# B3zaleel/draco-sharp

Hardware: AMD Instinct MI355X
Metric: decoded_meshes_per_sec (higher is better)
Workload: dtype int32

## Files before the change

### draco-sharp_amd/csrc/dsa_api.hip

```cpp
#include <hip/hip_runtime.h>
#include <atomic>
#include <mutex>

#include <cstdarg>
#include <cstdio>
#include <cstring>
#include <memory>
#include <new>
#include <string>
#include <vector>

#include "../../include/draco_mi355x.h"
#include "dsa_kernels.h"
#include "dsa_seams.h"
#include "dsa_general.h"
#include "dsa_host_parse.h"
#include "dsa_host_util.h"

namespace {

enum { STG_LOCATE = 0, STG_CONNECTIVITY, STG_TRAVERSE, STG_OPERANDS, STG_SYMBOLS, STG_PREDICT, STG_FINALIZE, STG_TOTAL };
static const char *kStageNames[DSA_NUM_STAGES] = {"locate", "connectivity", "traverse", "para_operands",
                                                 "symbols", "predict", "finalize", "total"};
enum { KT_CHAIN = 0, KT_CONNECTIVITY, KT_TRAVERSE, KT_SYMBOLS_EARLY, KT_SYMBOLS_LATE, KT_OCT_STREAMS, KT_PREDICT_WRAP_EARLY, KT_PREDICT_WRAP_LATE, KT_FACES,
       KT_SEAM_TABLES, KT_TRAVERSE_ATT, KT_TEXCOORDS, KT_COUNT };
static const char *kKernelNames[KT_COUNT] = {"k_chain", "k_connectivity", "k_traverse", "k_symbols_reg[early]", "k_symbols_reg[late]", "k_predict_oct_streams",
                                             "k_predict_wrap[early]", "k_predict_wrap[late]", "k_faces", "k_seam_tables", "k_traverse_att", "k_texcoords"};


}

struct EncLane {
  int device = 0;
  hipStream_t st = nullptr;
  hostutil::Staging stage[2];
  int next = 0;
  hostutil::UploadTurns *upload_turn = nullptr;
  uint32_t upload_chunk = 0;
  hipStream_t walk_st = nullptr;
  hipEvent_t tables_done = nullptr, walk_done = nullptr;
  hipEvent_t seams_done = nullptr;
  struct Buf {
    void *p = nullptr; uint64_t cap = 0;
    hipError_t ensure(uint64_t bytes) {
      if (bytes <= cap) return hipSuccess;
      if (p) (void)hipFree(p);
      p = nullptr; cap = 0;
      const uint64_t want = bytes + bytes / 4;
      hipError_t e = hipMalloc(&p, want);
      if (e != hipSuccess) { (void)hipGetLastError(); p = nullptr; e = hipMalloc(&p, bytes); if (e == hipSuccess) cap = bytes; else p = nullptr; return e; }
      cap = want;
      return hipSuccess;
    }
    ~Buf() { if (p) (void)hipFree(p); }
  } arena, streams, conns, seams, packed, items;
  ~EncLane() {
    if (walk_st) { (void)hipStreamSynchronize(walk_st); (void)hipStreamDestroy(walk_st); }
    if (st) { (void)hipStreamSynchronize(st); (void)hipStreamDestroy(st); }
    if (tables_done) (void)hipEventDestroy(tables_done);
    if (walk_done) (void)hipEventDestroy(walk_done);
    if (seams_done) (void)hipEventDestroy(seams_done);
  }
};

struct StreamSet {
  hipStream_t stream = nullptr;
  hipStream_t stream2 = nullptr;
  hipStream_t stream3 = nullptr;
  hipStream_t stream4 = nullptr;
  hipStream_t stream5 = nullptr;
  hipEvent_t ev_join3 = nullptr, ev_trav = nullptr, ev_maps = nullptr, ev_early = nullptr, ev_flips = nullptr;
  hipEvent_t ev_fork = nullptr, ev_join = nullptr, ev_conn = nullptr;
  hipEvent_t ev_seambits = nullptr, ev_tables = nullptr, ev_att = nullptr;
  hipEvent_t ev_pred = nullptr;
  bool own_stream = false;
  hipError_t create(hipStream_t user, int least, int greatest) {
    hipError_t e = hipSuccess;
    if (user) { stream = user; own_stream = false; }
    else { e = hipStreamCreateWithPriority(&stream, hipStreamNonBlocking, greatest); own_stream = e == hipSuccess; }
    if (e == hipSuccess) e = hipStreamCreateWithPriority(&stream4, hipStreamNonBlocking, (least + greatest) / 2);
    if (e == hipSuccess) e = hipStreamCreateWithPriority(&stream2, hipStreamNonBlocking, least);
    if (e == hipSuccess) e = hipStreamCreateWithFlags(&stream3, hipStreamNonBlocking);
    if (e == hipSuccess) e = hipStreamCreateWithPriority(&stream5, hipStreamNonBlocking, least);
    for (hipEvent_t *ev : {&ev_join3, &ev_trav, &ev_maps, &ev_flips, &ev_early, &ev_fork, &ev_join, &ev_conn, &ev_seambits, &ev_tables, &ev_att, &ev_pred})
      if (e == hipSuccess) e = hipEventCreateWithFlags(ev, hipEventDisableTiming);
    return e;
  }
  void destroy() {
    for (hipEvent_t *ev : {&ev_join3, &ev_trav, &ev_maps, &ev_flips, &ev_early, &ev_fork, &ev_join, &ev_conn, &ev_seambits, &ev_tables, &ev_att, &ev_pred}) { if (*ev) (void)hipEventDestroy(*ev); *ev = nullptr; }
    for (hipStream_t *s : {&stream2, &stream3, &stream4, &stream5}) { if (*s) (void)hipStreamDestroy(*s); *s = nullptr; }
    if (own_stream && stream) (void)hipStreamDestroy(stream);
    stream = nullptr;
  }
};

struct dsa_context {
  int device = 0;
  StreamSet sets[2];
  int num_sets = 0;
  bool set1_made = false;
  int prio_least = 0, prio_greatest = 0;
  int last_set = 0;
  hipEvent_t last_done = nullptr;
  hipStream_t up = nullptr;
  hipStream_t down = nullptr;
  bool profiling = false;
  std::string err;
  hostutil::Staging stage[2];
  int stage_next = 0;
  struct Spare { uint8_t *p; uint64_t bytes; };
  std::vector<Spare> spare_arenas, spare_mirrors, spare_descs, spare_packed;
  static constexpr size_t kSpares = 3;
  std::atomic<int> live_batches{0};
  std::atomic<bool> doomed{false};
  std::mutex mu;
  std::vector<std::unique_ptr<EncLane>> enc_lanes;
  bool gate_ok = false;
  std::string gate_note;
};

struct dsa_batch {
  dsa_context *ctx = nullptr;
  uint32_t n = 0;
  std::vector<MeshLayout> layouts;
  std::vector<HostMesh> host;
  std::vector<MeshDesc> descs;
  uint8_t *arena = nullptr;
  uint64_t arena_bytes = 0, arena_cap = 0;
  MeshLayout *d_layouts = nullptr;
  MeshDesc *d_descs = nullptr;
  BatchGlobals *d_globals = nullptr;
  BatchGlobals globals = {};
  uint64_t out_base = 0, out_bytes = 0;
  uint64_t out_values = 0, out_values_bytes = 0;
  std::vector<CompactMesh> compact;
  CompactMesh *d_compact = nullptr;
  uint64_t packed_bytes = 0;
  uint8_t *d_packed = nullptr;
  uint64_t d_packed_cap = 0;
  bool mirror_compact = false;
  uint32_t max_faces = 0, max_vertices = 0, max_atts = 0, max_att_data = 0;
  uint64_t sum_vertices = 0;
  bool any_general = false, any_valence = false, any_seamed = false, any_multipara = false;
  bool decoded = false, collected = false;
  hipEvent_t ev[DSA_NUM_STAGES + 1] = {};
  hipEvent_t ev_sym[2] = {};
  hipEvent_t ev_k[KT_COUNT][2] = {};
  bool k_timed[KT_COUNT] = {};
  bool have_events = false;
  float stage_ms[DSA_NUM_STAGES] = {};
  float kernel_ms[KT_COUNT] = {};
  hipEvent_t ev_uploaded = nullptr, ev_done = nullptr, ev_descs = nullptr, ev_down = nullptr;
  MeshDesc *descs_pin = nullptr;
  uint64_t descs_pin_bytes = 0;
  uint8_t *mirror = nullptr;
  uint64_t mirror_bytes = 0;
  bool mirror_owned = false, download_queued = false, downloaded = false;
  bool all_general = false;
  dsa_batch *retry = nullptr;
  std::vector<int32_t> retry_index;
};

namespace {

dsa_status set_err(dsa_context *ctx, dsa_status st, const char *fmt, ...) {
  if (ctx) {
    char buf[512];
    va_list ap;
    va_start(ap, fmt);
    vsnprintf(buf, sizeof(buf), fmt, ap);
    va_end(ap);
// ... 176 lines not shown
  HIP_TRY(ctx, hipEventCreateWithFlags(&b->ev_done, hipEventDisableTiming));
  HIP_TRY(ctx, hipEventCreateWithFlags(&b->ev_descs, hipEventDisableTiming));
  HIP_TRY(ctx, hipEventCreateWithFlags(&b->ev_down, hipEventDisableTiming));
  {
    const uint64_t need = sizeof(MeshDesc) * (uint64_t)(n ? n : 1);
    uint8_t *p = take_spare(ctx, ctx->spare_descs, need, &b->descs_pin_bytes);
    if (!p) { HIP_TRY(ctx, hipHostMalloc((void **)&p, need + need / 2, hipHostMallocDefault)); b->descs_pin_bytes = need + need / 2; }
    b->descs_pin = (MeshDesc *)p;
  }
  {
    int turn;
    { std::lock_guard<std::mutex> g(ctx->mu); turn = ctx->stage_next; ctx->stage_next ^= 1; }
    hostutil::Staging &stg = ctx->stage[turn];
    HIP_TRY(ctx, stg.acquire(upload_bytes));
    uint8_t *h = stg.buf.p;
    if (n) memcpy(h + off_layouts, b->layouts.data(), sizeof(MeshLayout) * (size_t)n);
    memset(h + sizeof(MeshLayout) * (size_t)n, 0, (size_t)(off_globals - sizeof(MeshLayout) * (uint64_t)n));
    memcpy(h + off_globals, &b->globals, sizeof(BatchGlobals));
    const uint64_t first = n ? b->layouts[0].stream : upload_bytes;
    memset(h + off_globals + sizeof(BatchGlobals), 0, (size_t)(first - off_globals - sizeof(BatchGlobals)));
    if (n) memcpy(h + off_compact, b->compact.data(), sizeof(CompactMesh) * (size_t)n);
    hostutil::parallel_for(n, [&](uint32_t i) {
      const uint64_t at = b->layouts[i].stream, end = at + lengths[i], next = i + 1 < n ? b->layouts[i + 1].stream : upload_bytes;
      if (lengths[i]) memcpy(h + at, streams[i], lengths[i]);
      memset(h + end, 0, (size_t)(next - end));
    }, 8);
    HIP_TRY(ctx, hipMemcpyAsync(b->arena, h, upload_bytes, hipMemcpyHostToDevice, ctx->up));
    HIP_TRY(ctx, stg.submitted(ctx->up));
    HIP_TRY(ctx, hipEventRecord(b->ev_uploaded, ctx->up));
  }
  guard.b = nullptr;
  *out = b;
  return DSA_OK;
}

void gate_check(dsa_context *c) {
  hipFuncAttributes chain{}, reg{}, gate{};
  if (hipFuncGetAttributes(&chain, (const void *)dsa::k_chain) != hipSuccess || hipFuncGetAttributes(&reg, (const void *)dsa::k_symbols_reg) != hipSuccess ||
      hipFuncGetAttributes(&gate, (const void *)dsa::k_register_gate) != hipSuccess) {
    (void)hipGetLastError();
    c->gate_ok = false; c->gate_note = "k_register_gate left out: kernel attributes not available";
    return;
  }
  auto up8 = [](int r) { return (r + 7) / 8 * 8; };
  const int rc = up8(chain.numRegs), rr = up8(reg.numRegs), rg = up8(gate.numRegs), simd = 512;
  const int left = simd - 4 * rc - 3 * rr;
  c->gate_ok = left >= 0 && rg > left && rr > left && rg <= left + 3 * rr;
  char buf[256];
  snprintf(buf, sizeof(buf), "k_register_gate %s: registers k_chain %d, k_symbols_reg %d, k_register_gate %d; %d left beside 4 + 3 waves of a SIMD",
           c->gate_ok ? "in use" : "left out", chain.numRegs, reg.numRegs, gate.numRegs, left);
  c->gate_note = buf;
}

}

extern "C" {

int dsa_abi_version(void) { return DSA_ABI_VERSION; }

int dsa_device_count(void) {
  int n = 0;
  if (hipGetDeviceCount(&n) != hipSuccess) return 0;
  return n;
}

dsa_status dsa_context_create(int device, void *stream, dsa_context **out) {
  if (!out) return DSA_ERR_INVALID_ARGUMENT;
  *out = nullptr;
  int n = 0;
  if (hipGetDeviceCount(&n) != hipSuccess || device < 0 || device >= n) return DSA_ERR_DEVICE;
  dsa_context *c = new (std::nothrow) dsa_context();
  if (!c) return DSA_ERR_OUT_OF_MEMORY;
  c->device = device;
  if (hipSetDevice(device) != hipSuccess) { delete c; return DSA_ERR_DEVICE; }
  int least = 0, greatest = 0;
  (void)hipDeviceGetStreamPriorityRange(&least, &greatest);
  c->num_sets = stream ? 1 : 2;
  c->prio_least = least; c->prio_greatest = greatest;
  if (c->sets[0].create((hipStream_t)stream, least, greatest) != hipSuccess) { dsa_context_destroy(c); return DSA_ERR_DEVICE; }
  if (hipStreamCreateWithFlags(&c->up, hipStreamNonBlocking) != hipSuccess ||
      hipStreamCreateWithFlags(&c->down, hipStreamNonBlocking) != hipSuccess ||
      hipEventCreateWithFlags(&c->last_done, hipEventDisableTiming) != hipSuccess) { dsa_context_destroy(c); return DSA_ERR_DEVICE; }
  gate_check(c);
  *out = c;
  return DSA_OK;
}

void dsa_context_destroy(dsa_context *ctx) {
  if (!ctx) return;
  {
    std::lock_guard<std::mutex> g(ctx->mu);
    if (ctx->live_batches.load() > 0) { ctx->doomed = true; return; }
  }
  (void)hipSetDevice(ctx->device);
  if (ctx->up) { (void)hipStreamSynchronize(ctx->up); (void)hipStreamDestroy(ctx->up); }
  if (ctx->down) { (void)hipStreamSynchronize(ctx->down); (void)hipStreamDestroy(ctx->down); }
  drop_spares(ctx, ctx->spare_arenas, false);
  drop_spares(ctx, ctx->spare_packed, false);
  drop_spares(ctx, ctx->spare_mirrors, true);
  drop_spares(ctx, ctx->spare_descs, true);
  for (StreamSet &set : ctx->sets) set.destroy();
  if (ctx->last_done) (void)hipEventDestroy(ctx->last_done);
  delete ctx;
}

const char *dsa_last_error(const dsa_context *ctx) { return ctx ? ctx->err.c_str() : "null context"; }

dsa_status dsa_context_set_profiling(dsa_context *ctx, int enabled) {
  if (!ctx) return DSA_ERR_INVALID_ARGUMENT;
  ctx->profiling = enabled != 0;
  return DSA_OK;
}

#define DSA_GUARD(ctx, expr)                                                                              \
  try { return (expr); }                                                                                   \
  catch (const std::bad_alloc &) { return set_err((ctx), DSA_ERR_OUT_OF_MEMORY, "host allocation failed"); } \
  catch (...) { return set_err((ctx), DSA_ERR_DEVICE, "unexpected failure inside the library"); }

dsa_status dsa_batch_create(dsa_context *ctx, uint32_t n, const uint8_t *const *streams, const size_t *lengths, dsa_batch **out) {
  DSA_GUARD(ctx, build_batch(ctx, n, streams, lengths, out));
}

static dsa_status create_packed(dsa_context *ctx, uint32_t n, const uint8_t *blob, const uint64_t *offsets, dsa_batch **out) {
  std::vector<const uint8_t *> ptrs(n);
  std::vector<size_t> lens(n);
  for (uint32_t i = 0; i < n; ++i) {
    if (offsets[i + 1] < offsets[i]) return set_err(ctx, DSA_ERR_INVALID_ARGUMENT, "offsets must be non-decreasing");
    ptrs[i] = blob + offsets[i];
    lens[i] = (size_t)(offsets[i + 1] - offsets[i]);
  }
  return build_batch(ctx, n, ptrs.data(), lens.data(), out);
}
dsa_status dsa_batch_create_packed(dsa_context *ctx, uint32_t n, const uint8_t *blob, const uint64_t *offsets, dsa_batch **out) {
  if (!ctx || !out || (n && (!blob || !offsets))) return set_err(ctx, DSA_ERR_INVALID_ARGUMENT, "null argument");
  DSA_GUARD(ctx, create_packed(ctx, n, blob, offsets, out));
}

dsa_status dsa_batch_decode(dsa_batch *b) {
  if (!b) return DSA_ERR_INVALID_ARGUMENT;
  dsa_context *ctx = b->ctx;
  HIP_TRY(ctx, hipSetDevice(ctx->device));
  const uint32_t n = b->n;
  const bool was_decoded = b->decoded;
  b->decoded = true;
  b->collected = false;
  if (b->retry) { dsa_batch_free(b->retry); b->retry = nullptr; }
  b->retry_index.clear();
  int set_turn = 0;
  {
    std::lock_guard<std::mutex> g(ctx->mu);
    if (ctx->num_sets > 1 && ctx->last_done && hipEventQuery(ctx->last_done) == hipErrorNotReady) {
      set_turn = ctx->last_set ^ 1;
      if (set_turn == 1 && !ctx->set1_made) {
        if (ctx->sets[1].create(nullptr, ctx->prio_least, ctx->prio_greatest) == hipSuccess) ctx->set1_made = true;
        else { (void)hipGetLastError(); ctx->sets[1].destroy(); set_turn = 0; }
      }
    }
    (void)hipGetLastError();
    ctx->last_set = set_turn;
  }
  StreamSet &S = ctx->sets[set_turn];
  hipStream_t st = S.stream;
  if (n == 0) {
    HIP_TRY(ctx, hipEventRecord(b->ev_done, st));
    HIP_TRY(ctx, hipEventRecord(b->ev_descs, st));
    return DSA_OK;
  }
  const bool prof = ctx->profiling;
  if (prof && !b->have_events) {
    for (int i = 0; i <= DSA_NUM_STAGES; ++i) HIP_TRY(ctx, hipEventCreate(&b->ev[i]));
    for (int i = 0; i < 2; ++i) HIP_TRY(ctx, hipEventCreate(&b->ev_sym[i]));
    for (int k = 0; k < KT_COUNT; ++k) for (int i = 0; i < 2; ++i) HIP_TRY(ctx, hipEventCreate(&b->ev_k[k][i]));
    b->have_events = true;
  }
  for (int k = 0; k < KT_COUNT; ++k) b->k_timed[k] = false;
  auto k_begin = [&](int k, hipStream_t s) { if (prof && !b->k_timed[k]) (void)hipEventRecord(b->ev_k[k][0], s); };
  auto k_end = [&](int k, hipStream_t s) { if (prof && !b->k_timed[k]) { (void)hipEventRecord(b->ev_k[k][1], s); b->k_timed[k] = true; } };
  int evi = 0;
  auto mark = [&]() -> hipError_t { return prof ? hipEventRecord(b->ev[evi++], st) : hipSuccess; };
  if (b->download_queued && !b->downloaded) HIP_TRY(ctx, hipStreamWaitEvent(st, b->ev_down, 0));
  if (was_decoded) HIP_TRY(ctx, hipStreamWaitEvent(st, b->ev_done, 0));
  b->download_queued = false; b->downloaded = false;
  HIP_TRY(ctx, hipStreamWaitEvent(st, b->ev_uploaded, 0));
  HIP_TRY(ctx, hipMemsetAsync(b->d_descs, 0, sizeof(MeshDesc) * n, st));
  HIP_TRY(ctx, hipMemsetAsync(&b->d_globals->pool_cursor, 0, sizeof(unsigned long long) * 2, st));
  HIP_TRY(ctx, mark());
  {
    uint32_t gx = std::max<uint32_t>(1, std::min<uint32_t>((b->max_faces + 16383) / 16384, 4));
    hipLaunchKernelGGL(dsa::k_init, dim3(gx, n), dim3(256), 0, st, b->arena, b->d_layouts, n);
  }
  hipLaunchKernelGGL(dsa::k_locate, dim3(n), dim3(WAVE), 0, st, b->arena, b->d_layouts, b->d_descs, n, b->d_globals);
  for (uint32_t r = 0; r < std::max<uint32_t>(1, b->max_atts); ++r) {
    hipLaunchKernelGGL(dsa::k_tags, dim3(n), dim3(WAVE), 0, st, b->arena, b->d_layouts, b->d_descs, n);
    hipLaunchKernelGGL(dsa::k_locate_resume, dim3(n), dim3(WAVE), 0, st, b->arena, b->d_layouts, b->d_descs, n, b->d_globals);
  }
  if (b->any_valence) hipLaunchKernelGGL(dsa::k_valence_lists, dim3(n, 6), dim3(WAVE), 0, st, b->arena, b->d_layouts, b->d_descs, n);
  HIP_TRY(ctx, mark());
  const uint32_t na = std::max<uint32_t>(1, b->max_atts);
  static const bool serial = getenv("DSA_SERIAL") != nullptr;
#ifdef DSA_EXPERIMENTS
  auto env_int = [](const char *name, int dflt) { const char *e = getenv(name); return e ? atoi(e) : dflt; };
  static const int fuse_choice = env_int("DSA_FUSE_OPERANDS", -1), chain_choice = env_int("DSA_CHAIN", -1);
  static const uint32_t lane_flags = (uint32_t)env_int("DSA_LANES", (int)PW_FLAG);
  static const bool run_window = env_int("DSA_TRAV_NO_WINDOW", 0) == 0;
  static const int trav_split = env_int("DSA_TRAV_SPLIT", 1), split_mode = env_int("DSA_SYM_SPLIT", 1);
  static const uint32_t wide_flag = env_int("DSA_SYM_WIDE", 1) ? SYM_WIDE : 0u;
  static const bool early_fuse_on = env_int("DSA_EARLY_FUSE", 0) != 0;
  static const uint32_t oct_lpw = (uint32_t)env_int("DSA_OCT_LPW", 16);
  static const bool handoff_on = env_int("DSA_LATE_HANDOFF", 0) != 0;
#else
  const bool handoff_on = false;
  const int fuse_choice = -1, chain_choice = -1, trav_split = 1, split_mode = 1;
  const uint32_t lane_flags = PW_FLAG, wide_flag = SYM_WIDE;
  const bool run_window = true, early_fuse_on = false;
#endif
  const int oct_choice = []() { const char *e = getenv("DSA_OCT_STREAMS"); return e ? atoi(e) : -1; }();
  const bool oct_rule = n >= 3584 && (uint64_t)b->max_vertices * n <= 4 * b->sum_vertices;
  const uint32_t oct_flag = (oct_choice >= 0 ? oct_choice != 0 : oct_rule) && !(lane_flags & (LN_FLAG_OCT | LN_FLAG_PREDICT)) ? OS_FLAG : 0u;
  hipStream_t st2 = serial ? st : S.stream2, st3 = serial ? st : S.stream3;
  HIP_TRY(ctx, hipEventRecord(S.ev_fork, st));
  HIP_TRY(ctx, hipStreamWaitEvent(st2, S.ev_fork, 0));
  if (b->any_general) {
    HIP_TRY(ctx, hipStreamWaitEvent(st3, S.ev_fork, 0));
    hipLaunchKernelGGL(dsa::k_general, dim3(n), dim3(WAVE), 0, st3, b->arena, b->d_layouts, b->d_descs, n);
    hipLaunchKernelGGL(dsa::k_general_tables, dim3(n), dim3(WAVE), 0, st3, b->arena, b->d_layouts, b->d_descs, n);
    hipLaunchKernelGGL(dsa::k_general_attributes<0>, dim3(n), dim3(WAVE), 0, st3, b->arena, b->d_layouts, b->d_descs, n);
    hipLaunchKernelGGL(dsa::k_general_attributes<1>, dim3(n), dim3(WAVE), 0, st3, b->arena, b->d_layouts, b->d_descs, n);
    if (n > 2048) hipLaunchKernelGGL(dsa::k_general_values_crowded, dim3(n), dim3(WAVE), 0, st3, b->arena, b->d_layouts, b->d_descs, n);
    else hipLaunchKernelGGL(dsa::k_general_attributes<2>, dim3(n), dim3(WAVE), 0, st3, b->arena, b->d_layouts, b->d_descs, n);
    hipLaunchKernelGGL(dsa::k_general_attributes<3>, dim3(n), dim3(WAVE), 0, st3, b->arena, b->d_layouts, b->d_descs, n);
    HIP_TRY(ctx, hipEventRecord(S.ev_join3, st3));
  }
  if (!b->any_general) HIP_TRY(ctx, hipStreamWaitEvent(st3, S.ev_fork, 0));
  {
    uint32_t lpm = 1;
    while (lpm < b->max_att_data) lpm *= 2;
    const uint32_t per_wave = WAVE / lpm;
    hipLaunchKernelGGL(dsa::k_conn_checks, dim3((n + per_wave - 1) / per_wave), dim3(WAVE), 0, st3, b->arena, b->d_layouts, b->d_descs, n, lpm);
// ... 43 lines not shown
    k_end(KT_CONNECTIVITY, st);
    if (!b->any_seamed) HIP_TRY(ctx, launch_faces());
    if (b->any_seamed) {
      HIP_TRY(ctx, hipEventRecord(S.ev_trav, st));
      HIP_TRY(ctx, hipStreamWaitEvent(st3, S.ev_trav, 0));
      k_begin(KT_SEAM_TABLES, st3);
      hipLaunchKernelGGL(dsa::k_seam_tables, dim3(n), dim3(WAVE), 0, st3, b->arena, b->d_layouts, b->d_descs, n);
      k_end(KT_SEAM_TABLES, st3);
      for (uint32_t r = 0; r < std::max<uint32_t>(1, b->max_atts); ++r) {
        hipLaunchKernelGGL(dsa::k_tags, dim3(n), dim3(WAVE), 0, st3, b->arena, b->d_layouts, b->d_descs, n);
        hipLaunchKernelGGL(dsa::k_locate_resume, dim3(n), dim3(WAVE), 0, st3, b->arena, b->d_layouts, b->d_descs, n, b->d_globals);
      }
      HIP_TRY(ctx, hipEventRecord(S.ev_tables, st3));
      k_begin(KT_TRAVERSE_ATT, st3);
      hipLaunchKernelGGL(dsa::k_traverse_att, dim3(n, std::max<uint32_t>(1, b->max_att_data)), dim3(WAVE), 0, st3, b->arena, b->d_layouts, b->d_descs, n);
      k_end(KT_TRAVERSE_ATT, st3);
      HIP_TRY(ctx, hipEventRecord(S.ev_att, st3));
      HIP_TRY(ctx, launch_faces());
      {
        uint32_t lpm = 1;
        while (lpm < na) lpm *= 2;
        const uint32_t per_wave = WAVE / lpm;
        hipStream_t st5 = serial ? st : S.stream5;
        HIP_TRY(ctx, hipStreamWaitEvent(st5, S.ev_tables, 0));
        hipLaunchKernelGGL(dsa::k_flip_bits, dim3((n + per_wave - 1) / per_wave), dim3(WAVE), 0, st5, b->arena, b->d_layouts, b->d_descs, n, lpm, 1u);
        hipLaunchKernelGGL(dsa::k_orient_bits, dim3((n + per_wave - 1) / per_wave), dim3(WAVE), 0, st5, b->arena, b->d_layouts, b->d_descs, n, lpm, 1u);
        HIP_TRY(ctx, hipEventRecord(S.ev_flips, st5));
      }
    }
    HIP_TRY(ctx, mark());
    const uint32_t per = (n + (uint32_t)trav_split - 1) / (uint32_t)trav_split;
    k_begin(KT_TRAVERSE, st);
    for (uint32_t m0 = 0; m0 < n; m0 += per) {
      const uint32_t cnt = std::min(per, n - m0);
      hipLaunchKernelGGL(dsa::k_traverse, dim3(cnt), dim3(WAVE), 0, st, b->arena, b->d_layouts + m0, b->d_descs + m0, cnt, trav_flags);
    }
    k_end(KT_TRAVERSE, st);
    if (b->any_seamed) {
      HIP_TRY(ctx, launch_seam_maps());
    }
  }
  HIP_TRY(ctx, mark());
  if (prof) HIP_TRY(ctx, hipEventRecord(b->ev_sym[0], st2));
#ifdef DSA_EXPERIMENTS
  if (lane_flags & LN_FLAG_SYMBOLS) {
    const uint32_t groups = (n + WAVE - 1) / WAVE;
    hipLaunchKernelGGL(dsa::lanes::k_symbols_lanes<LN_T2_SYMS>, dim3(groups, na), dim3(WAVE), 0, st2, b->arena, b->d_layouts, b->d_descs, n, lane_flags);
    hipLaunchKernelGGL(dsa::lanes::k_symbols_lanes<LN_T1_SYMS>, dim3(groups, na), dim3(WAVE), 0, st2, b->arena, b->d_layouts, b->d_descs, n, lane_flags);
    hipLaunchKernelGGL(dsa::lanes::k_symbols_lanes<LN_T0_SYMS>, dim3(groups, na), dim3(WAVE), 0, st2, b->arena, b->d_layouts, b->d_descs, n, lane_flags);
  }
#endif
  const bool sym_split = !serial && !(lane_flags & (LN_FLAG_SYMBOLS | LN_FLAG_PREDICT)) && split_mode != 0;
  hipStream_t st4 = sym_split ? S.stream4 : st2;
  auto launch_symbols = [&](hipStream_t s, uint32_t fl, bool gate = false) {
    fl |= wide_flag;
    const uint32_t tier_blocks = (uint32_t)std::min<uint64_t>((uint64_t)n * na, SYM_TIER_BLOCKS);
    if (wide_flag) hipLaunchKernelGGL(dsa::k_symbols_wide, dim3(n, na), dim3(WAVE), 0, s, b->arena, b->d_layouts, b->d_descs, n, fl);
    hipLaunchKernelGGL(dsa::k_symbols<1>, dim3(tier_blocks), dim3(WAVE), dsa::sym_tier_lds_bytes(1), s, b->arena, b->d_layouts, b->d_descs, n, na, fl);
    hipLaunchKernelGGL(dsa::k_symbols<0>, dim3(tier_blocks), dim3(WAVE), dsa::sym_tier_lds_bytes(0), s, b->arena, b->d_layouts, b->d_descs, n, na, fl);
    hipLaunchKernelGGL(dsa::k_symbols<2>, dim3(tier_blocks), dim3(WAVE), dsa::sym_tier_lds_bytes(2), s, b->arena, b->d_layouts, b->d_descs, n, na, fl);
    if (gate) hipLaunchKernelGGL(dsa::k_register_gate, dim3(SYM_TIER_BLOCKS), dim3(WAVE), 0, s);
    const int kt = (fl & SYM_EARLY_ONLY) ? KT_SYMBOLS_EARLY : KT_SYMBOLS_LATE;
    k_begin(kt, s);
    hipLaunchKernelGGL(dsa::k_symbols_reg, dim3(n, na), dim3(WAVE), 0, s, b->arena, b->d_layouts, b->d_descs, n, fl);
    k_end(kt, s);
  };
  {
    const uint32_t gx = std::max<uint32_t>(1, std::min<uint32_t>((b->max_vertices + 16383) / 16384, 4));
    hipLaunchKernelGGL(dsa::k_point_maps, dim3(gx, n), dim3(256), 0, st2, b->arena, b->d_layouts, b->d_descs, n);
    HIP_TRY(ctx, hipEventRecord(S.ev_conn, st2));
  }
  const uint32_t early_fuse = early_fuse_on && !(lane_flags & (LN_FLAG_PREDICT | LN_FLAG_OCT)) ? SYM_EARLY_FUSE : 0u;
  const uint32_t hand = handoff ? LATE_HANDOFF : 0u;
  if (sym_split && split_mode == 2) {
    launch_symbols(st2, lane_flags | SYM_EARLY_ONLY | early_fuse);
    HIP_TRY(ctx, hipEventRecord(S.ev_conn, st2));
    HIP_TRY(ctx, hipStreamWaitEvent(st4, S.ev_conn, 0));
    launch_symbols(st2, lane_flags | SYM_LATE_ONLY | hand);
  } else if (sym_split && oct_flag) {
    HIP_TRY(ctx, hipStreamWaitEvent(st4, S.ev_conn, 0));
    launch_symbols(st4, lane_flags | SYM_EARLY_ONLY | early_fuse);
    launch_symbols(st2, lane_flags | SYM_LATE_ONLY | hand, ctx->gate_ok);
  } else if (sym_split) {
    HIP_TRY(ctx, hipStreamWaitEvent(st4, S.ev_conn, 0));
    launch_symbols(st4, lane_flags | SYM_EARLY_ONLY | early_fuse);
    launch_symbols(st2, lane_flags | SYM_LATE_ONLY | hand);
  } else launch_symbols(st2, lane_flags | early_fuse | hand);
  if (b->any_seamed) {
    HIP_TRY(ctx, hipEventRecord(S.ev_pred, st2));
    HIP_TRY(ctx, hipStreamWaitEvent(st2, S.ev_tables, 0));
    launch_symbols(st2, lane_flags | SYM_CORNER);
  }
  if (prof) HIP_TRY(ctx, hipEventRecord(b->ev_sym[1], st2));
  HIP_TRY(ctx, hipEventRecord(S.ev_join, st2));
#ifdef DSA_EXPERIMENTS
  if (lane_flags & LN_FLAG_PREDICT) hipLaunchKernelGGL(dsa::lanes::k_predict_lanes<16>, dim3((n + 15) / 16, na), dim3(WAVE), 0, st4, b->arena, b->d_layouts, b->d_descs, n, 0u);
  else
#endif
  {
    if (oct_flag) {
      k_begin(KT_OCT_STREAMS, st4);
      hipLaunchKernelGGL(dsa::k_predict_oct_streams, dim3((n + WAVE - 1) / WAVE, na), dim3(WAVE), OS_RING * 1024u, st4, b->arena, b->d_layouts, b->d_descs, n);
      k_end(KT_OCT_STREAMS, st4);
    }
    hipLaunchKernelGGL(dsa::k_predict, dim3(n, na), dim3(WAVE), 0, st4, b->arena, b->d_layouts, b->d_descs, n, 0u, lane_flags | oct_flag);
    if (lane_flags & PW_FLAG) {
      k_begin(KT_PREDICT_WRAP_EARLY, st4);
      hipLaunchKernelGGL(dsa::k_predict_wrap, dim3(n, na), dim3(WAVE), 0, st4, b->arena, b->d_layouts, b->d_descs, n, 0u, lane_flags);
      k_end(KT_PREDICT_WRAP_EARLY, st4);
    }
#ifdef DSA_EXPERIMENTS
    if (lane_flags & LN_FLAG_OCT) {
      if (oct_lpw == 8) hipLaunchKernelGGL(dsa::lanes::k_predict_oct_lanes<8>, dim3((n + 7) / 8, na), dim3(WAVE), 0, st4, b->arena, b->d_layouts, b->d_descs, n, lane_flags);
      else if (oct_lpw == 32) hipLaunchKernelGGL(dsa::lanes::k_predict_oct_lanes<32>, dim3((n + 31) / 32, na), dim3(WAVE), 0, st4, b->arena, b->d_layouts, b->d_descs, n, lane_flags);
      else if (oct_lpw == 64) hipLaunchKernelGGL(dsa::lanes::k_predict_oct_lanes<64>, dim3((n + 63) / 64, na), dim3(WAVE), 0, st4, b->arena, b->d_layouts, b->d_descs, n, lane_flags);
      else hipLaunchKernelGGL(dsa::lanes::k_predict_oct_lanes<16>, dim3((n + 15) / 16, na), dim3(WAVE), 0, st4, b->arena, b->d_layouts, b->d_descs, n, lane_flags);
    }
#endif
// ... 524 lines not shown
```

### draco-sharp_amd/csrc/dsa_kernels.h

```cpp
#pragma once
#include <hip/hip_runtime.h>
#include <stdint.h>

#include "dsa_common.h"
#include "dsa_locate.h"
#ifdef DSA_EXPERIMENTS
#include "dsa_lanes.h"
#else
#define LN_FLAG_SYMBOLS 1u
#define LN_FLAG_PREDICT 2u
#define LN_FLAG_OCT 8u
namespace dsa { namespace lanes {
__device__ __forceinline__ bool ln_sym_eligible(const AttrDesc &, const MeshLayout &, uint32_t, uint32_t) { return false; }
__device__ __forceinline__ bool ln_oct_eligible(const AttrDesc &, uint32_t) { return false; }
} }
#endif

#ifndef DSA_CHAIN_PRIO
#define DSA_CHAIN_PRIO 3
#endif

namespace dsa {

__device__ __forceinline__ uint32_t cnext(uint32_t c) { return (c % 3u == 2u) ? c - 2u : c + 1u; }
__device__ __forceinline__ uint32_t cprev(uint32_t c) { return (c % 3u == 0u) ? c + 2u : c - 1u; }
__device__ __forceinline__ uint32_t uni(uint32_t v) { return (uint32_t)__builtin_amdgcn_readfirstlane((int)v); }
__device__ __forceinline__ uint32_t lane_id() { return threadIdx.x & 63u; }
template <class T>
__device__ __forceinline__ T *uni_ptr(T *p) {
  const uint64_t v = (uint64_t)p;
  return (T *)(((uint64_t)(uint32_t)__builtin_amdgcn_readfirstlane((int)(uint32_t)(v >> 32)) << 32) | (uint32_t)__builtin_amdgcn_readfirstlane((int)(uint32_t)v));
}
__device__ __forceinline__ uint32_t rdlane(uint32_t v, uint32_t l) { return (uint32_t)__builtin_amdgcn_readlane((int)v, (int)l); }
#define SYM_WIDE 0x800u
#define SYM_EARLY_ONLY 0x100u
#define SYM_LATE_ONLY 0x200u
#define SYM_CORNER 0x1000u
#define PRED_FRONT 0x10000u
#define PRED_BEHIND 0x20000u
__device__ __forceinline__ bool att_behind_tables(const AttrDesc &a) { return a.corner_data != 0 || a.late_located != 0; }
__device__ __forceinline__ bool att_is_late(const AttrDesc &a) { return (a.have_scheme && a.pred_kind != 0) || att_behind_tables(a); }
#define PW_FLAG 4u
#define LATE_HANDOFF 0x40000u
__device__ __forceinline__ void late_handoff(uint8_t *arena, const MeshLayout &L, MeshDesc *D, uint32_t ai, uint32_t flags, uint32_t bit);
__device__ __forceinline__ bool pred_filtered(const AttrDesc &a, uint32_t flags) {
  return ((flags & PRED_FRONT) && att_behind_tables(a)) || ((flags & PRED_BEHIND) && !att_behind_tables(a));
}
__device__ __forceinline__ bool sym_filtered(const AttrDesc &a, uint32_t flags) {
  if (att_behind_tables(a)) return !(flags & SYM_CORNER);
  if (flags & SYM_CORNER) return true;
  const bool late = a.have_scheme && a.pred_kind != 0;
  return ((flags & SYM_EARLY_ONLY) && late) || ((flags & SYM_LATE_ONLY) && !late);
}
__device__ __forceinline__ uint64_t clk() { return __builtin_amdgcn_s_memtime(); }
__device__ __forceinline__ uint64_t realclk() { return __builtin_amdgcn_s_memrealtime(); }
__device__ __forceinline__ uint32_t leading_lanes(bool pred) { uint64_t m = ~__ballot(pred); return m ? (uint32_t)__builtin_ctzll(m) : 64u; }
#define WAIT_VM0() __builtin_amdgcn_s_waitcnt(0x0F70)

template <int CTRL>
__device__ __forceinline__ uint32_t dpp_mov(uint32_t x) { return (uint32_t)__builtin_amdgcn_update_dpp(0, (int)x, CTRL, 0xF, 0xF, false); }
__device__ __forceinline__ uint32_t lane_prev(uint32_t x) { return dpp_mov<0x138>(x); }
template <class Op>
__device__ __forceinline__ uint32_t wave_incl_scan(uint32_t x, Op op) {
  const uint32_t lane = lane_id(), rl = lane & 15u;
  uint32_t t;
  t = dpp_mov<0x111>(x); if (rl >= 1) x = op(t, x);
  t = dpp_mov<0x112>(x); if (rl >= 2) x = op(t, x);
  t = dpp_mov<0x114>(x); if (rl >= 4) x = op(t, x);
  t = dpp_mov<0x118>(x); if (rl >= 8) x = op(t, x);
  t = dpp_mov<0x142>(x); if ((lane & 31u) >= 16) x = op(t, x);
  t = dpp_mov<0x143>(x); if (lane >= 32) x = op(t, x);
  return x;
}
__device__ __forceinline__ uint32_t wave_excl_scan(uint32_t v, uint32_t *total) {
  const uint32_t x = wave_incl_scan(v, [](uint32_t a, uint32_t b) { return a + b; });
  *total = rdlane(x, 63);
  return x - v;
}

template <bool CP> struct Rec;
struct FaceIds { uint32_t v0, v1, v2, o0, o1, o2; };
template <> struct Rec<false> {
  static constexpr uint32_t WORDS = 8;
  struct Raw { uint4 v, o; };
  static __device__ __forceinline__ Raw load(const uint32_t *frec, uint32_t f) { Raw r; r.v = ((const uint4 *)frec)[(size_t)f * 2]; r.o = ((const uint4 *)frec)[(size_t)f * 2 + 1]; return r; }
// ... 1811 lines not shown
          }
        }
      } else {
        const uint32_t xs = uni((uint32_t)(P >> 32));
        mine = (lane == j) ? xs : mine;
        const uint32_t k5 = (xs >> 6) & 31u, l6 = xs & 63u;
        const uint32_t e0 = rdlane(tab_lo[k5], l6), e1 = rdlane(tab_hi[k5], l6);
        const uint32_t e = (xs & 2048u) ? e1 : e0;
        P = (uint64_t)((e & 0xFFFFu) * (xs >> 12) + (e >> 16)) << 32;
        ++j;
      }
    }
    if (lane < cnt) out[i0 + lane] = mine;
  }
  WAIT_VM0();
  __syncthreads();
  if (VLIST) {
    for (uint32_t i = lane; i < num_values; i += WAVE) out[i] = slot_sym[out[i] & 4095u];
    WAIT_VM0();
    __syncthreads();
    if (lane == 0) atomicOr(&D->val_lists_done, 1u << ai);
    return;
  }
  if (TAGS) {
    uint8_t *tags = arena + L.out[ai];
    uint64_t bits = 0;
    uint32_t worst = 0;
    const uint32_t nc = a.nc_portable;
    for (uint32_t i = lane; i < num_values; i += WAVE) {
      const uint32_t v = slot_sym[out[i] & 4095u];
      tags[i] = (uint8_t)v;
      bits += (uint64_t)v * nc;
      worst = v > worst ? v : worst;
    }
    for (int d = 32; d >= 1; d >>= 1) {
      bits += ((uint64_t)(uint32_t)__shfl_xor((int)(uint32_t)(bits >> 32), d, WAVE) << 32) | (uint32_t)__shfl_xor((int)(uint32_t)bits, d, WAVE);
      const uint32_t w2 = (uint32_t)__shfl_xor((int)worst, d, WAVE);
      worst = w2 > worst ? w2 : worst;
    }
    WAIT_VM0();
    __syncthreads();
    if (lane == 0) { a.table = (bits & 0x00FFFFFFFFFFFFFFull) | ((uint64_t)(worst > 255u ? 255u : worst) << 56); a.tags_done = 1; }
    return;
  }
  const bool positive = a.have_scheme && (a.pred_transform == 2 || a.pred_transform == 3);
  for (uint32_t i = lane; i < num_values; i += WAVE) {
    uint32_t v = slot_sym[out[i] & 4095u];
    out[i] = positive ? v : ((v & 1u) ? (uint32_t)(-(int32_t)(v >> 1) - 1) : (v >> 1));
  }
  early_tail(arena, L, D, ai, flags);
  late_handoff(arena, L, D, ai, flags, 1u);
}

__global__ __launch_bounds__(WAVE, 6) void k_symbols_reg(uint8_t *arena, const MeshLayout *layouts, MeshDesc *descs, uint32_t n, uint32_t flags) {
  uint32_t mesh = blockIdx.x, ai = blockIdx.y;
  if (mesh >= n) return;
  MeshDesc *D = &descs[mesh];
  if (D->status != ST_OK || D->general || ai >= D->num_attributes) return;
  reg_decode_stream<REG_ATTR>(arena, layouts[mesh], D, ai, flags);
}
__global__ __launch_bounds__(WAVE, 6) void k_tags(uint8_t *arena, const MeshLayout *layouts, MeshDesc *descs, uint32_t n) {
  uint32_t mesh = blockIdx.x;
  if (mesh >= n) return;
  MeshDesc *D = &descs[mesh];
  if (D->status != ST_OK || D->general || !D->values_pending || D->resume_att >= D->num_attributes) return;
  if (D->values_pending == 2) return;
  reg_decode_stream<REG_TAGS>(arena, layouts[mesh], D, D->resume_att, 0u);
}
__global__ __launch_bounds__(WAVE, 6) void k_valence_lists(uint8_t *arena, const MeshLayout *layouts, MeshDesc *descs, uint32_t n) {
  uint32_t mesh = blockIdx.x, c = blockIdx.y;
  if (mesh >= n) return;
  MeshDesc *D = &descs[mesh];
  if (D->status != ST_OK || D->general || D->encoder_type == 0 || D->traversal_type != 2) return;
  reg_decode_stream<REG_VLIST>(arena, layouts[mesh], D, c, 0u);
}

__device__ __forceinline__ bool sym_reg_eligible(const AttrDesc &a, const MeshLayout &L, uint32_t ai) {
  return a.source == SRC_RAW && a.precision_bits == 12 && a.num_symbols <= REG_MAX_SYMS && a.num_distinct > 1 &&
         L.out_cap[ai] >= 4096 * 6 + REG_MAX_SYMS * 4;
}
__device__ __forceinline__ bool sym_wide_eligible(const AttrDesc &a, const MeshLayout &L, uint32_t ai) {
  if (a.source != SRC_RAW || a.num_distinct <= 1 || sym_reg_eligible(a, L, ai)) return false;
  const bool compact = a.num_symbols > SYM_MAX_LDS;
  const uint32_t nse = compact ? a.num_distinct : a.num_symbols;
  if (nse <= 64 || nse > WIDE_MAX_SYMS || a.precision_bits > 16) return false;
  return compact ? (a.table != 0 && 2ull * nse + 1 <= (unsigned long long)a.num_symbols + 2) : (L.out_cap[ai] >= 4ull * (nse + 1));
}

__global__ __launch_bounds__(WAVE) void k_symbols_wide(uint8_t *arena, const MeshLayout *layouts, MeshDesc *descs, uint32_t n, uint32_t flags) {
  const uint32_t mesh = blockIdx.x, ai = blockIdx.y;
  if (mesh >= n) return;
  MeshDesc *D = &descs[mesh];
  if (D->status != ST_OK || D->general || ai >= D->num_attributes) return;
  const MeshLayout &L = layouts[mesh];
  const AttrDesc &a = D->att[ai];
  if (a.source == SRC_BYTES) return;
  if (lanes::ln_sym_eligible(a, L, ai, flags)) return;
  if (sym_filtered(a, flags)) return;
  if (!sym_wide_eligible(a, L, ai)) return;
  const uint32_t lane = lane_id();
  const uint32_t num_values = a.num_entries * a.nc_portable;
  if (num_values == 0) return;
  const uint8_t *stream = arena + L.stream;
  const uint32_t stream_len = L.stream_len;
  uint32_t *out = (uint32_t *)(arena + L.work[ai]);
  const bool compact = a.num_symbols > SYM_MAX_LDS;
  const uint32_t nsym = compact ? a.num_distinct : a.num_symbols;
  uint32_t *symtab = compact ? (uint32_t *)(arena + a.table) : nullptr;
  uint32_t *gtab = compact ? symtab + nsym : (uint32_t *)(arena + L.out[ai]);
  const uint32_t P = a.precision_bits, precision = 1u << P, l_base = precision * 4;
  if (lane == 0) {
    Rd r(stream, stream_len, a.off_table);
    uint32_t k = 0;
    bool ok = true;
    for (uint32_t i = 0; i < a.num_symbols && ok; ++i) {
      const uint32_t pd = r.u8(), token = pd & 3u;
      if (token == 3u) {
        const uint32_t offset = pd >> 2;
        if (i + offset >= a.num_symbols) ok = false;
        if (!compact) for (uint32_t j = 0; j <= offset && i + j < a.num_symbols; ++j) gtab[i + j] = 0;
        i += offset;
      } else {
        uint32_t pr = pd >> 2;
        for (uint32_t j = 0; j < token; ++j) pr |= r.u8() << (8 * (j + 1) - 2);
        if (compact) { if (pr) { if (k >= nsym) ok = false; else { gtab[k] = pr; symtab[k] = i; ++k; } } }
        else gtab[i] = pr;
      }
    }
    if (!ok || !r.ok || (compact && k != nsym)) fail(D, ST_INVALID, 400);
    WAIT_VM0();
    __threadfence_block();
  }
  __syncthreads();
// ... 1016 lines not shown
```

### draco-sharp_amd/csrc/dsa_types.h

```cpp
#pragma once
#include <stdint.h>

#define DSA_MAX_ATT 16
#define DSA_MAX_ATT_DATA 15
#define DSA_INVALID 0xFFFFFFFFu

#define ST_OK 0
#define ST_INVALID 1
#define ST_NOTIMPL 2
#define DSA_SITE_RETRY_GENERAL 170

#define SRC_TAGGED 0
#define SRC_RAW 1
#define SRC_FIXED 2
#define SRC_BYTES 3

struct AttrDesc {
  uint8_t att_type, data_type, nc, normalized;
  uint8_t seq_type;
  int8_t decoder_id;
  int8_t pred_method;
  int8_t pred_kind;
  int8_t pred_transform;
  uint8_t nc_portable;
// ... 147 lines not shown
  uint64_t total;
};
#if defined(__HIPCC__)
__host__ __device__
#endif
inline SeamLayout seam_layout(uint64_t F, uint64_t V, uint64_t A, bool compact) {
  SeamLayout g;
  const uint64_t NVA = 3 * F;
  uint64_t cur = 0;
  auto take = [&](uint64_t bytes) { uint64_t at = cur; cur = (cur + bytes + 16 + 255) & ~255ull; return at; };
  g.eseam = take(4 * F);
  g.vseam = take(V);
  g.pbase = take(4 * V);
  g.data = cur;
  cur = 0;
  g.bits = take(4 * ((3 * F / 2 + 31) / 32 + 4));
  g.rec = take((compact ? 16 : 32) * F);
  g.vbase = take(4 * V);
  g.vflag = take(NVA);
  g.d2c = take(4 * NVA);
  g.v2d = take(4 * NVA);
  g.fvis = take(F);
  g.stack = take(4 * F);
  g.para = take(12 * NVA);
  g.orient = take(4 * (NVA / 32 + 1));
  g.data_stride = cur;
  g.total = g.data + A * g.data_stride;
  return g;
}

struct MpPrep { uint32_t id[4][3]; };
#define MP_FOUND_SHIFT 29u
#define MP_ID_MASK 0x1FFFFFFFu

struct TcPrep {
  uint32_t next_id, prev_id;
  int64_t pn_norm2;
  int64_t cn_dot_pn;
  int64_t norm;
  double inv;
};

struct CompactMesh {
  uint64_t faces;
  uint32_t u16, pad;
  uint64_t map[DSA_MAX_ATT];
};

struct BatchGlobals {
  uint64_t pool;
  uint64_t pool_bytes;
  unsigned long long pool_cursor;
  unsigned long long pad;
};

struct MeshLayout {
  uint64_t stream;
  uint32_t stream_len;
  uint32_t cap_faces;
  uint32_t cap_vertices;
  uint32_t cap_attributes;
  uint64_t frec;
  uint64_t vrec;
  uint64_t d2c;
  uint64_t v2d;
  uint64_t fvis, vvis;
  uint64_t fstamp, vstamp;
  uint64_t splits;
  uint32_t cap_splits;
  uint32_t rec_compact;
  uint64_t vrank;
  uint64_t para;
  uint64_t faces;
  uint64_t work[DSA_MAX_ATT];
  uint64_t out[DSA_MAX_ATT];
  uint64_t map[DSA_MAX_ATT];
  uint32_t work_cap[DSA_MAX_ATT];
  uint32_t out_cap[DSA_MAX_ATT];
  uint64_t gen;
  uint64_t gen_bytes;
  uint32_t cap_points;
  uint32_t pad2;
  uint64_t seam;
  uint64_t seam_bytes;
  uint64_t tc[DSA_MAX_ATT];
  uint32_t mp_att;
  uint32_t pad_mp;
};
```

Before: 105,700.

## Add opt-in LDS-table rANS symbol decoder sharing work via atomic cursor

Adds a k_symbols_lds kernel that builds the rANS slot table in LDS and decodes streams one wave at a time. It runs on a new low-priority stream alongside k_symbols_reg, and both claim (mesh, attribute) items from a shared per-leg atomic cursor in BatchGlobals. The LDS path is gated by an environment variable plus register and LDS budget checks. The register decoder now always claims its work through the atomic cursor rather than using block indices, which adds one atomic per block and extra event waits.

```diff
diff --git a/draco-sharp_amd/csrc/dsa_api.hip b/draco-sharp_amd/csrc/dsa_api.hip
--- a/draco-sharp_amd/csrc/dsa_api.hip
+++ b/draco-sharp_amd/csrc/dsa_api.hip
@@ -69,10 +69,12 @@
   hipStream_t stream3 = nullptr;
   hipStream_t stream4 = nullptr;
   hipStream_t stream5 = nullptr;
+  hipStream_t stream6 = nullptr;
   hipEvent_t ev_join3 = nullptr, ev_trav = nullptr, ev_maps = nullptr, ev_early = nullptr, ev_flips = nullptr;
   hipEvent_t ev_fork = nullptr, ev_join = nullptr, ev_conn = nullptr;
   hipEvent_t ev_seambits = nullptr, ev_tables = nullptr, ev_att = nullptr;
   hipEvent_t ev_pred = nullptr;
+  hipEvent_t ev_lds[3] = {};
   bool own_stream = false;
   hipError_t create(hipStream_t user, int least, int greatest) {
     hipError_t e = hipSuccess;
@@ -82,13 +84,14 @@
     if (e == hipSuccess) e = hipStreamCreateWithPriority(&stream2, hipStreamNonBlocking, least);
     if (e == hipSuccess) e = hipStreamCreateWithFlags(&stream3, hipStreamNonBlocking);
     if (e == hipSuccess) e = hipStreamCreateWithPriority(&stream5, hipStreamNonBlocking, least);
-    for (hipEvent_t *ev : {&ev_join3, &ev_trav, &ev_maps, &ev_flips, &ev_early, &ev_fork, &ev_join, &ev_conn, &ev_seambits, &ev_tables, &ev_att, &ev_pred})
+    if (e == hipSuccess) e = hipStreamCreateWithPriority(&stream6, hipStreamNonBlocking, least);
+    for (hipEvent_t *ev : {&ev_join3, &ev_trav, &ev_maps, &ev_flips, &ev_early, &ev_fork, &ev_join, &ev_conn, &ev_seambits, &ev_tables, &ev_att, &ev_pred, &ev_lds[0], &ev_lds[1], &ev_lds[2]})
       if (e == hipSuccess) e = hipEventCreateWithFlags(ev, hipEventDisableTiming);
     return e;
   }
   void destroy() {
-    for (hipEvent_t *ev : {&ev_join3, &ev_trav, &ev_maps, &ev_flips, &ev_early, &ev_fork, &ev_join, &ev_conn, &ev_seambits, &ev_tables, &ev_att, &ev_pred}) { if (*ev) (void)hipEventDestroy(*ev); *ev = nullptr; }
-    for (hipStream_t *s : {&stream2, &stream3, &stream4, &stream5}) { if (*s) (void)hipStreamDestroy(*s); *s = nullptr; }
+    for (hipEvent_t *ev : {&ev_join3, &ev_trav, &ev_maps, &ev_flips, &ev_early, &ev_fork, &ev_join, &ev_conn, &ev_seambits, &ev_tables, &ev_att, &ev_pred, &ev_lds[0], &ev_lds[1], &ev_lds[2]}) { if (*ev) (void)hipEventDestroy(*ev); *ev = nullptr; }
+    for (hipStream_t *s : {&stream2, &stream3, &stream4, &stream5, &stream6}) { if (*s) (void)hipStreamDestroy(*s); *s = nullptr; }
     if (own_stream && stream) (void)hipStreamDestroy(stream);
     stream = nullptr;
   }
@@ -117,6 +120,8 @@
   std::vector<std::unique_ptr<EncLane>> enc_lanes;
   bool gate_ok = false;
   std::string gate_note;
+  bool lds_ok = false;
+  uint32_t lds_blocks = 0;
 };
 
 struct dsa_batch {
@@ -399,6 +404,27 @@
   c->gate_note = buf;
 }
 
+void lds_check(dsa_context *c) {
+  hipFuncAttributes chain{}, reg{}, lds{};
+  hipDeviceProp_t prop{};
+  c->lds_ok = false;
+  if (hipFuncGetAttributes(&chain, (const void *)dsa::k_chain) != hipSuccess || hipFuncGetAttributes(&reg, (const void *)dsa::k_symbols_reg) != hipSuccess ||
+      hipFuncGetAttributes(&lds, (const void *)dsa::k_symbols_lds) != hipSuccess || hipGetDeviceProperties(&prop, c->device) != hipSuccess) {
+    (void)hipGetLastError();
+    c->gate_note += "; k_symbols_lds left out: kernel attributes not available";
+    return;
+  }
+  auto up8 = [](int r) { return (r + 7) / 8 * 8; };
+  const int left = 512 - 4 * up8(chain.numRegs) - 3 * up8(reg.numRegs);
+  const long cu_lds = 160 * 1024, chain_lds = 16 * ((long)chain.sharedSizeBytes + CN_LDS_WORDS * 4), own_lds = 4 * ((long)lds.sharedSizeBytes + SL_LDS_BYTES);
+  c->lds_ok = up8(lds.numRegs) <= left && chain_lds + own_lds <= cu_lds && prop.multiProcessorCount > 0;
+  c->lds_blocks = 4u * (uint32_t)std::max(prop.multiProcessorCount, 1);
+  char buf[256];
+  snprintf(buf, sizeof(buf), "; k_symbols_lds %s: %d registers for %d left beside 4 + 3 waves of a SIMD, %ld + %ld bytes of LDS per CU", c->lds_ok ? "in use" : "left out",
+           lds.numRegs, left, chain_lds, own_lds);
+  c->gate_note += buf;
+}
+
 }
 
 extern "C" {
@@ -429,6 +455,7 @@
       hipStreamCreateWithFlags(&c->down, hipStreamNonBlocking) != hipSuccess ||
       hipEventCreateWithFlags(&c->last_done, hipEventDisableTiming) != hipSuccess) { dsa_context_destroy(c); return DSA_ERR_DEVICE; }
   gate_check(c);
+  lds_check(c);
   *out = c;
   return DSA_OK;
 }
@@ -530,7 +557,7 @@
   b->download_queued = false; b->downloaded = false;
   HIP_TRY(ctx, hipStreamWaitEvent(st, b->ev_uploaded, 0));
   HIP_TRY(ctx, hipMemsetAsync(b->d_descs, 0, sizeof(MeshDesc) * n, st));
-  HIP_TRY(ctx, hipMemsetAsync(&b->d_globals->pool_cursor, 0, sizeof(unsigned long long) * 2, st));
+  HIP_TRY(ctx, hipMemsetAsync(&b->d_globals->pool_cursor, 0, sizeof(BatchGlobals) - offsetof(BatchGlobals, pool_cursor), st));
   HIP_TRY(ctx, mark());
   {
     uint32_t gx = std::max<uint32_t>(1, std::min<uint32_t>((b->max_faces + 16383) / 16384, 4));
@@ -680,6 +707,12 @@
 #endif
   const bool sym_split = !serial && !(lane_flags & (LN_FLAG_SYMBOLS | LN_FLAG_PREDICT)) && split_mode != 0;
   hipStream_t st4 = sym_split ? S.stream4 : st2;
+  const int lds_choice = []() { const char *e = getenv("DSA_SYM_LDS"); return e ? atoi(e) : 0; }();
+  const bool lds_able = ctx->lds_ok && !early_fuse_on && !handoff_on && !(lane_flags & (LN_FLAG_SYMBOLS | LN_FLAG_PREDICT));
+  const bool lds_rule = n >= 3584 && chain && !serial && split_mode == 1;
+  const int sym_lds = !lds_able || lds_choice <= 0 ? 0 : lds_choice == 2 ? 2 : !lds_rule ? 0 : lds_choice == 3 ? 3 : 1;
+  hipStream_t st6 = serial ? st : S.stream6;
+  bool lds_forked = false;
   auto launch_symbols = [&](hipStream_t s, uint32_t fl, bool gate = false) {
     fl |= wide_flag;
     const uint32_t tier_blocks = (uint32_t)std::min<uint64_t>((uint64_t)n * na, SYM_TIER_BLOCKS);
@@ -688,10 +721,20 @@
     hipLaunchKernelGGL(dsa::k_symbols<0>, dim3(tier_blocks), dim3(WAVE), dsa::sym_tier_lds_bytes(0), s, b->arena, b->d_layouts, b->d_descs, n, na, fl);
     hipLaunchKernelGGL(dsa::k_symbols<2>, dim3(tier_blocks), dim3(WAVE), dsa::sym_tier_lds_bytes(2), s, b->arena, b->d_layouts, b->d_descs, n, na, fl);
     if (gate) hipLaunchKernelGGL(dsa::k_register_gate, dim3(SYM_TIER_BLOCKS), dim3(WAVE), 0, s);
+    const int leg = (fl & SYM_CORNER) ? 2 : (fl & SYM_EARLY_ONLY) ? 0 : 1;
+    const bool lds_leg = sym_lds && !(sym_lds == 3 && leg == 0);
+    if (lds_leg) {
+      if (!lds_forked || leg == 2) (void)hipStreamWaitEvent(st6, leg == 2 ? S.ev_tables : S.ev_conn, 0);
+      lds_forked = true;
+      const uint32_t reserve = sym_lds == 2 ? 0u : 3u * ctx->lds_blocks;
+      hipLaunchKernelGGL(dsa::k_symbols_lds, dim3(ctx->lds_blocks), dim3(WAVE), SL_LDS_BYTES, st6, b->arena, b->d_layouts, b->d_descs, n, na, fl, b->d_globals, reserve);
+      (void)hipEventRecord(S.ev_lds[leg], st6);
+    }
     const int kt = (fl & SYM_EARLY_ONLY) ? KT_SYMBOLS_EARLY : KT_SYMBOLS_LATE;
     k_begin(kt, s);
-    hipLaunchKernelGGL(dsa::k_symbols_reg, dim3(n, na), dim3(WAVE), 0, s, b->arena, b->d_layouts, b->d_descs, n, fl);
+    if (sym_lds != 2) hipLaunchKernelGGL(dsa::k_symbols_reg, dim3(n, na), dim3(WAVE), 0, s, b->arena, b->d_layouts, b->d_descs, n, fl, b->d_globals);
     k_end(kt, s);
+    if (lds_leg) (void)hipStreamWaitEvent(s, S.ev_lds[leg], 0);
   };
   {
     const uint32_t gx = std::max<uint32_t>(1, std::min<uint32_t>((b->max_vertices + 16383) / 16384, 4));
diff --git a/draco-sharp_amd/csrc/dsa_kernels.h b/draco-sharp_amd/csrc/dsa_kernels.h
--- a/draco-sharp_amd/csrc/dsa_kernels.h
+++ b/draco-sharp_amd/csrc/dsa_kernels.h
@@ -3,6 +3,7 @@
 #include <stdint.h>
 
 #include "dsa_common.h"
+#include "dsa_symbols_lds.h"
 #include "dsa_locate.h"
 #ifdef DSA_EXPERIMENTS
 #include "dsa_lanes.h"
@@ -31,6 +32,7 @@
   const uint64_t v = (uint64_t)p;
   return (T *)(((uint64_t)(uint32_t)__builtin_amdgcn_readfirstlane((int)(uint32_t)(v >> 32)) << 32) | (uint32_t)__builtin_amdgcn_readfirstlane((int)(uint32_t)v));
 }
+__device__ __forceinline__ uint64_t uni64(uint64_t v) { return ((uint64_t)uni((uint32_t)(v >> 32)) << 32) | uni((uint32_t)v); }
 __device__ __forceinline__ uint32_t rdlane(uint32_t v, uint32_t l) { return (uint32_t)__builtin_amdgcn_readlane((int)v, (int)l); }
 #define SYM_WIDE 0x800u
 #define SYM_EARLY_ONLY 0x100u
@@ -1948,9 +1950,17 @@
   late_handoff(arena, L, D, ai, flags, 1u);
 }
 
-__global__ __launch_bounds__(WAVE, 6) void k_symbols_reg(uint8_t *arena, const MeshLayout *layouts, MeshDesc *descs, uint32_t n, uint32_t flags) {
-  uint32_t mesh = blockIdx.x, ai = blockIdx.y;
-  if (mesh >= n) return;
+__device__ __forceinline__ uint32_t sym_leg(uint32_t flags) { return (flags & SYM_CORNER) ? 2u : (flags & SYM_EARLY_ONLY) ? 0u : 1u; }
+__device__ __forceinline__ uint32_t sym_claim(BatchGlobals *G, uint32_t flags) {
+  uint32_t item = 0;
+  if (lane_id() == 0) item = atomicAdd(&G->sym_cursor[sym_leg(flags)], 1u);
+  return uni(item);
+}
+
+__global__ __launch_bounds__(WAVE, 6) void k_symbols_reg(uint8_t *arena, const MeshLayout *layouts, MeshDesc *descs, uint32_t n, uint32_t flags, BatchGlobals *G) {
+  const uint32_t item = sym_claim(G, flags);
+  if (item >= n * gridDim.y) return;
+  const uint32_t ai = item / n, mesh = item - ai * n;
   MeshDesc *D = &descs[mesh];
   if (D->status != ST_OK || D->general || ai >= D->num_attributes) return;
   reg_decode_stream<REG_ATTR>(arena, layouts[mesh], D, ai, flags);
@@ -1975,6 +1985,115 @@
   return a.source == SRC_RAW && a.precision_bits == 12 && a.num_symbols <= REG_MAX_SYMS && a.num_distinct > 1 &&
          L.out_cap[ai] >= 4096 * 6 + REG_MAX_SYMS * 4;
 }
+#define SL_LDS_BYTES 16384u
+template <class T>
+__device__ __forceinline__ T &sl_at(T *base, uint32_t byte_off) { return *(T *)((uint8_t *)base + byte_off); }
+struct SlWave {
+  const uint32_t *tab;
+  const uint32_t *abuf;
+  uint32_t *out;
+  uint32_t lane, W, mine;
+  __device__ __forceinline__ uint32_t uni(uint32_t v) const { return dsa::uni(v); }
+  __device__ __forceinline__ uint32_t table(uint32_t slot) const { return tab[slot]; }
+  __device__ __forceinline__ void window(uint32_t chunk) { W = sl_at(abuf, (chunk * 64u + lane) * 4u); }
+  __device__ __forceinline__ uint32_t dword(uint32_t l) const { return rdlane(W, l); }
+  __device__ __forceinline__ void park(uint32_t j, uint32_t slot) { mine = lane == j ? slot : mine; }
+  __device__ __forceinline__ void flush(uint32_t i0, uint32_t cnt) { if (lane < cnt) sl_at(out, (i0 + lane) * 4u) = mine; }
+};
+__device__ __forceinline__ void lds_decode_stream(uint8_t *arena, const MeshLayout &L, MeshDesc *D, uint32_t ai, uint32_t flags, uint32_t *tab) {
+  AttrDesc &a = D->att[ai];
+  if (lanes::ln_sym_eligible(a, L, ai, flags)) return;
+  if (sym_filtered(a, flags)) return;
+  if (!sym_reg_eligible(a, L, ai)) return;
+  uint8_t *scratch = arena + uni64(L.out[ai]);
+  uint32_t *out = (uint32_t *)(arena + uni64(L.work[ai]));
+  const uint64_t stream_at = uni64(L.stream);
+  const uint8_t *stream = arena + stream_at;
+  const uint32_t stream_len = uni(L.stream_len), off_table = uni(a.off_table), size_rans = uni(a.size_rans);
+  const bool positive = uni(a.have_scheme && (a.pred_transform == 2 || a.pred_transform == 3) ? 1u : 0u) != 0;
+  uint32_t *slot_tab = (uint32_t *)scratch;
+  uint16_t *slot_sym = (uint16_t *)(scratch + 4096 * 4);
+  uint32_t *cumtab = (uint32_t *)(scratch + 4096 * 6);
+  const uint32_t lane = lane_id();
+  const uint32_t nsym = uni(a.num_symbols);
+  const uint32_t num_values = uni(a.num_entries * (uint32_t)a.nc_portable);
+  const uint32_t off_rans = uni(a.off_rans);
+  if (num_values == 0) return;
+  if (lane == 0) {
+    Rd r(stream, stream_len, off_table);
+    if (!read_prob_table(r, nsym, cumtab)) fail(D, ST_INVALID, 400);
+  }
+  __syncthreads();
+  if (status_of(D) != ST_OK) return;
+  uint32_t carry = 0;
+  bool over = false;
+#pragma clang loop unroll(disable) vectorize(disable) interleave(disable)
+  for (uint32_t b0 = 0; b0 < REG_MAX_SYMS; b0 += WAVE) {
+    const uint32_t i = b0 + lane;
+    const uint32_t pr = i < nsym ? sl_at(cumtab, i * 4u) : 0u;
+    if (pr > 4095) over = true;
+    uint32_t tot;
+    const uint32_t ex = wave_excl_scan(pr, &tot);
+    sl_at(cumtab, i * 4u) = (pr << 12) | ((carry + ex) & 4095u);
+    carry += tot;
+    if (carry > 4096) over = true;
+  }
+  if (__ballot(over) || carry != 4096) { if (lane == 0) fail(D, carry != 4096 ? ST_INVALID : ST_NOTIMPL, 401); return; }
+  __syncthreads();
+#pragma clang loop unroll(disable) vectorize(disable) interleave(disable)
+  for (uint32_t sy = lane; sy < nsym; sy += WAVE) {
+    const uint32_t e = sl_at(cumtab, sy * 4u), f = e >> 12, c = e & 4095u;
+#pragma clang loop unroll(disable) vectorize(disable) interleave(disable)
+    for (uint32_t j = 0; j < f; ++j) { sl_at(slot_tab, (c + j) * 4u) = f | (j << 16); sl_at(slot_sym, (c + j) * 2u) = (uint16_t)sy; }
+  }
+  WAIT_VM0();
+  __syncthreads();
+#pragma clang loop unroll(disable) vectorize(disable) interleave(disable)
+  for (uint32_t k = 0; k < 4096u; k += WAVE) tab[k + lane] = sl_at(slot_tab, (k + lane) * 4u);
+  __syncthreads();
+  uint32_t x, off;
+  {
+    uint32_t st = 0, o = 0;
+    const bool ok = rans_init(stream + off_rans, size_rans, 16384, &st, &o);
+    if (!ok) { if (lane == 0) fail(D, ST_INVALID, 402); return; }
+    x = uni(st); off = uni(o);
+  }
+  const uint32_t mis = (uint32_t)((stream_at + off_rans) & 3u);
+  SlWave w;
+  w.tab = tab;
+  w.abuf = (const uint32_t *)(arena + (stream_at + off_rans - mis));
+  w.out = out;
+  w.lane = lane; w.W = 0; w.mine = 0;
+  symlds::decode(w, x, off, mis, num_values);
+  WAIT_VM0();
+  __syncthreads();
+#pragma clang loop unroll(disable) vectorize(disable) interleave(disable)
+  for (uint32_t i = lane; i < num_values; i += WAVE) {
+    const uint32_t v = sl_at(slot_sym, (sl_at(out, i * 4u) & 4095u) * 2u);
+    sl_at(out, i * 4u) = positive ? v : ((v & 1u) ? (uint32_t)(-(int32_t)(v >> 1) - 1) : (v >> 1));
+  }
+}
+__global__ __launch_bounds__(WAVE) __attribute__((amdgpu_num_vgpr(8))) void k_symbols_lds(uint8_t *arena, const MeshLayout *layouts, MeshDesc *descs, uint32_t n, uint32_t na, uint32_t flags, BatchGlobals *G,
+                                                      uint32_t reserve) {
+  extern __shared__ uint32_t sl_tab[];
+  const uint32_t total = n * na;
+  uint32_t *cursor = &G->sym_cursor[sym_leg(flags)];
+  for (;;) {
+    uint32_t item = DSA_INVALID;
+    if (lane_id() == 0) {
+      const uint32_t at = __hip_atomic_load(cursor, __ATOMIC_RELAXED, __HIP_MEMORY_SCOPE_AGENT);
+      if (at < total && total - at > reserve) item = atomicAdd(cursor, 1u);
+    }
+    item = uni(item);
+    if (item >= total) return;
+    const uint32_t ai = uni(item / n), mesh = item - ai * n;
+    MeshDesc *D = &descs[mesh];
+    if (D->status != ST_OK || D->general || ai >= D->num_attributes) continue;
+    lds_decode_stream(arena, layouts[mesh], D, ai, flags, sl_tab);
+    __syncthreads();
+  }
+}
+
 __device__ __forceinline__ bool sym_wide_eligible(const AttrDesc &a, const MeshLayout &L, uint32_t ai) {
   if (a.source != SRC_RAW || a.num_distinct <= 1 || sym_reg_eligible(a, L, ai)) return false;
   const bool compact = a.num_symbols > SYM_MAX_LDS;
diff --git a/draco-sharp_amd/csrc/dsa_symbols_lds.h b/draco-sharp_amd/csrc/dsa_symbols_lds.h
--- /dev/null
+++ b/draco-sharp_amd/csrc/dsa_symbols_lds.h
@@ -0,0 +1,43 @@
+#pragma once
+#include <stdint.h>
+
+#if defined(__HIPCC__)
+#define DSA_SL_HD __host__ __device__ __forceinline__
+#else
+#define DSA_SL_HD inline
+#endif
+
+namespace dsa {
+namespace symlds {
+
+template <class Wave>
+DSA_SL_HD void decode(Wave &w, uint32_t x, uint32_t off, uint32_t mis, uint32_t num_values) {
+  uint32_t res = 0, rc = 0, chunk = 0x7FFFFFFFu;
+  for (uint32_t i0 = 0; i0 < num_values; i0 += 64u) {
+    const uint32_t cnt = num_values - i0 < 64u ? num_values - i0 : 64u;
+    for (uint32_t j = 0; j < cnt; ++j) {
+      while (x < 16384u) {
+        if (rc == 0) {
+          if (off == 0) break;
+          const uint32_t end = off + mis;
+          const uint32_t d = (end - 1u) >> 2, r = end - 4u * d, ch = d >> 6;
+          if (ch != chunk) { chunk = ch; w.window(ch); }
+          res = w.uni(w.dword(d & 63u) << (8u * (4u - r)));
+          rc = r < off ? r : off;
+          off -= rc;
+        }
+        x = (x << 8) | (res >> 24);
+        res <<= 8;
+        --rc;
+      }
+      const uint32_t slot = x & 4095u;
+      w.park(j, slot);
+      const uint32_t e = w.uni(w.table(slot));
+      x = (e & 0xFFFFu) * (x >> 12) + (e >> 16);
+    }
+    w.flush(i0, cnt);
+  }
+}
+
+}
+}
diff --git a/draco-sharp_amd/csrc/dsa_types.h b/draco-sharp_amd/csrc/dsa_types.h
--- a/draco-sharp_amd/csrc/dsa_types.h
+++ b/draco-sharp_amd/csrc/dsa_types.h
@@ -223,6 +223,7 @@
   uint64_t pool_bytes;
   unsigned long long pool_cursor;
   unsigned long long pad;
+  uint32_t sym_cursor[4];
 };
 
 struct MeshLayout {
```

After: 100,200. -5.2%, worse.
